# microsoft/tutel

Hardware: AMD Instinct MI355X
Metric: MoE-layer fwd tokens/sec, 4096 tok x H=2048 x E=64 top-2 (higher is better)
Workload: dtype bf16

## Files before the change

tutel_amd/csrc/expert_ffn.hip:

```cpp
#include <mutex>

#include "gemm_dev.h"

#define FFN_NQ 8
#define FFN_THREADS 256

struct FfnArgs {
  GemmArgs g[2];
  uint32_t *ctl;
  int xcc_queue;
  int prefetch;
  unsigned long long *dbg;
};

template <bool FL> static constexpr size_t ffn_lds_bytes() { return (size_t)3 * 3 * GL_STAGE * 2 + (FL ? 16384 : 16); }

template <typename V> __device__ __forceinline__ V ffn_uni(V v) {
  static_assert(sizeof(V) == 4 || sizeof(V) == 8 || sizeof(V) == 1, "scalar fields only");
  if constexpr (sizeof(V) == 8) {
    const unsigned long long b = __builtin_bit_cast(unsigned long long, v);
    const unsigned lo = (unsigned)__builtin_amdgcn_readfirstlane((int)(unsigned)b), hi = (unsigned)__builtin_amdgcn_readfirstlane((int)(b >> 32));
    return __builtin_bit_cast(V, ((unsigned long long)hi << 32) | lo);
  } else if constexpr (sizeof(V) == 4) {
    return __builtin_bit_cast(V, __builtin_amdgcn_readfirstlane(__builtin_bit_cast(int, v)));
// ... 2 lines not shown
  }
}
__device__ __forceinline__ GemmArgs ffn_pick(const GemmArgs &a0, const GemmArgs &a1, int ph) {
  GemmArgs p;
#define FFN_SEL(f) p.f = ffn_uni(ph ? a1.f : a0.f)
  FFN_SEL(A); FFN_SEL(a_stride_e); FFN_SEL(a_stride_w); FFN_SEL(a_rpw); FFN_SEL(lda);
  FFN_SEL(W); FFN_SEL(w_stride_e); FFN_SEL(ldw);
  FFN_SEL(bias); FFN_SEL(bias_stride_e);
  FFN_SEL(D); FFN_SEL(d_stride_e); FFN_SEL(d_stride_w); FFN_SEL(d_rpw); FFN_SEL(ldd);
  FFN_SEL(E_loc); FFN_SEL(R); FFN_SEL(N); FFN_SEL(K);
  FFN_SEL(row_counts); FFN_SEL(row_align);
  FFN_SEL(a_rows); FFN_SEL(a_rows_mod); FFN_SEL(a_zero); FFN_SEL(a_span_bytes);
  FFN_SEL(fits32); FFN_SEL(rot_on); FFN_SEL(sgather); FFN_SEL(d_store);
  FFN_SEL(fl_idx8); FFN_SEL(fl_n); FFN_SEL(fl_loc);
  FFN_SEL(ntm); FFN_SEL(ntn); FFN_SEL(act_rt);
#undef FFN_SEL
  p.mul = nullptr; p.d_peer = nullptr; p.d_peer_off = 0;
  p.d_can = PeerCanary{nullptr, 0, 0, 0};
  p.sk_ws = nullptr; p.sk_flags = nullptr;
  return p;
}

__device__ __forceinline__ int ffn_queue_items(int q, int E, int nt1, int nt2, int *n1) {
  const int ne = q < E ? (E - q + FFN_NQ - 1) / FFN_NQ : 0;
  *n1 = ne * nt1;
  return ne * (nt1 + nt2);
}

struct FfnTail {
  uint32_t *tick;
  int q, tid;
  int *nxt, *snap;
  int on;
  __device__ __forceinline__ void operator()() const {
// ... 166 lines not shown
  if (mode <= 0) return TUTEL_AMD_ENOTSUP;
  const int E_loc = fc1.E_loc, dtype = fc1.dtype;
  if (E_loc <= 0 || fc1.R <= 0 || fc2.dtype != dtype) return TUTEL_AMD_ENOTSUP;
  FfnArgs a;
  int rc = tutel_gemm_args(fc1, &a.g[0]);
  if (rc != 0) return rc < 0 ? rc : TUTEL_AMD_ENOTSUP;
  rc = tutel_gemm_args(fc2, &a.g[1]);
  if (rc != 0) return rc < 0 ? rc : TUTEL_AMD_ENOTSUP;
  const bool fl = fc1.fl_idx8 != nullptr;
  if (!ffn_covers(a.g[0], a.g[1])) return TUTEL_AMD_ENOTSUP;
  if (fl && !(fc1.a_rows != nullptr && fc1.fl_n >= 1 && fc1.fl_n <= 15360 && E_loc <= 128 && fc1.K >= 2 * GL_BK && ((uintptr_t)fc1.fl_idx8 & 15) == 0 &&
              tutel_get_option(TUTEL_OPT_FUSED_LOCATION) != 0))
    return TUTEL_AMD_ENOTSUP;
  if (query) return 0;
  for (int i = 0; i < 2; ++i) {
    a.g[i].ntm = 1;
    a.g[i].ntn = (a.g[i].N + 255) / 256;
  }
  a.ctl = ffn_ctl(st, E_loc);
  if (a.ctl == nullptr) return TUTEL_AMD_ENOTSUP;
  a.xcc_queue = mode == 2 ? 0 : 1;
  a.prefetch = mode == 3 ? 0 : 1;
  a.dbg = g_ffn_dbg;
  const long long items = (long long)E_loc * (a.g[0].ntn + a.g[1].ntn);
  const int cus = ffn_cus();
  const int grid = (int)(items < cus ? items : cus);
  StageScope stage(TUTEL_STAGE_FC1, st);
  TUTEL_REQUIRE(act >= TUTEL_ACT_NONE && act <= TUTEL_ACT_SILU, "tutel_amd_expert_ffn: unknown activation %d", act);
  a.g[0].act_rt = act;
  a.g[1].act_rt = TUTEL_ACT_NONE;
  if (dtype == TUTEL_BF16) return fl ? ffn_launch_cfg<bf16_t, true>(a, grid, st) : ffn_launch_cfg<bf16_t, false>(a, grid, st);
  return fl ? ffn_launch_cfg<f16_t, true>(a, grid, st) : ffn_launch_cfg<f16_t, false>(a, grid, st);
// ... 27 lines not shown
```

tutel_amd/csrc/expert_gemm.hip:

```cpp
#include <stdlib.h>

#include <mutex>
#include <type_traits>

#include "common.h"

#include "gemm_dev.h"

template <typename T, bool W_KMAJOR, int ACT, bool NT, bool ROT, bool PACKED = false>
__global__ __launch_bounds__(GM_THREADS, 2) void expert_gemm_kernel(GemmArgs p) {
  constexpr int BK = 64, NBUF = 2;
  constexpr int LDK = BK + 8;
  constexpr int A_TILE = GM_BM * LDK;
  constexpr int W_TILE = W_KMAJOR ? GM_BN * LDK : BK * GM_LDN;
  constexpr int CPR = BK / 8;
  constexpr int RPP = GM_THREADS / CPR;
  constexpr int NLA = GM_BM / RPP;
  constexpr int NLW = W_KMAJOR ? GM_BN / RPP : BK / 16;
  extern __shared__ __attribute__((aligned(16))) unsigned char smem[];
  uint16_t *sA = reinterpret_cast<uint16_t *>(smem);
  uint16_t *sW = sA + NBUF * A_TILE;

  const int tid = threadIdx.x, lane = tid & 63, wid = tid >> 6;
  const int wm = wid >> 1, wn = wid & 1;
// ... 278 lines not shown
    GL_MMA(fa[2], fw[2]);
    GL_MMA(fa[3], fw[3]);

    __syncthreads();
  }
#undef GL_ISSUE
#undef GL_LOAD_FRAGS
#undef GL_MMA

  gemm_epilogue<T, ACT>(p, acc, bias_r, e, m0, n0, wm, wn, l31, kg, row_limit);
}

template <typename T, bool W_KMAJOR, int ACT, int NI, int NS, bool BUF = false, int BM = GB_BM, bool FL = false>
__global__ __launch_bounds__(BM * 2, 2) void expert_gemm_big_kernel(GemmArgs p) {
  extern __shared__ __attribute__((aligned(16))) unsigned char smem[];
  const int w = xcd_work_item(gridDim.x);
  gemm_big_tile<T, W_KMAJOR, ACT, NI, NS, BUF, BM, FL>(p, w / (p.ntm * p.ntn), w % p.ntm, (w / p.ntm) % p.ntn, smem);
}

#define PP_BUF (4 * GL_STAGE)

template <typename T, int ACT, bool W_ONCE, bool RAGGED = false, bool EARLY_BIAS = false, bool SPLITK = false, bool PACKED = false,
          bool GATE_UP = false>
__global__ __launch_bounds__(GB_THREADS, 2) void expert_gemm_pp_kernel(GemmArgs p) {
  extern __shared__ __attribute__((aligned(16))) unsigned char smem[];
  uint16_t *lds = reinterpret_cast<uint16_t *>(smem);

  const int tid = threadIdx.x, lane = tid & 63;
  const int wid = __builtin_amdgcn_readfirstlane(tid >> 6);
  const int wm = wid >> 1, wn = wid & 1;

  static_assert(!(PACKED && SPLITK), "the packed layout never splits K");
// ... 319 lines not shown
    (void)hipGetLastError();
    if (w) (void)hipFree(w);
    if (f) (void)hipFree(f);
    return false;
  }
  e->ws = w; e->flags = f; e->tiles = tiles;
  if (e == &g_sk[g_sk_n]) ++g_sk_n;
  *ws = w;
  *flags = f;
  return true;
}

template <typename T, int ACT>
static int launch_pp_splitk(const GemmArgs &a, hipStream_t st) {
  GemmArgs b = a;
  b.ntm = (a.R + GB_BM - 1) / GB_BM;
  b.ntn = (a.N + 255) / 256;
  const size_t tiles = (size_t)b.E_loc * b.ntm * b.ntn;
  const int nk = a.K / GL_BK;
  if (a.row_counts != nullptr || a.R % GB_BM != 0 || (nk & 1) || nk < 8 || (tiles & 3) || a.rot_on) return 1;
  if ((a.ldd & 7) || (a.d_stride_e & 7) || (a.d_stride_w & 7) || (reinterpret_cast<uintptr_t>(a.D) & 15)) return 1;
  if (!splitk_workspace(st, tiles, &b.sk_ws, &b.sk_flags)) return 1;
  return launch_lds(expert_gemm_pp_kernel<T, ACT, false, false, false, true>, (unsigned)(2 * tiles), GB_THREADS, PP_LDS_BYTES, st, b,
                    "tutel_amd_expert_gemm");
}

template <typename T, int ACT>
static int launch_pp(const GemmArgs &a, hipStream_t st) {
  GemmArgs b = a;
  b.ntm = (a.R + GB_BM - 1) / GB_BM;
  b.ntn = (a.N + 255) / 256;
  const int tail_rows = b.R % GB_BM;
  const bool ragged = b.row_counts != nullptr || (tail_rows != 0 && tail_rows <= GB_BM - 32);
  const bool early = tutel_get_option(TUTEL_OPT_GEMM_PERSIST) != 0;
  if (b.ntm == 1 && (long long)b.E_loc * b.ntn >= 256)
    return ragged ? launch_pp_cfg<T, ACT, true, true>(b, st) : (early ? launch_pp_cfg<T, ACT, true, false, true>(b, st) : launch_pp_cfg<T, ACT, true>(b, st));
  return ragged ? launch_pp_cfg<T, ACT, false, true>(b, st) : (early ? launch_pp_cfg<T, ACT, false, false, true>(b, st) : launch_pp_cfg<T, ACT, false>(b, st));
}

template <typename T, int ACT>
static int launch_pp_packed(const GemmArgs &a, int tiles_bound, hipStream_t st) {
  GemmArgs b = a;
  b.ntm = 1;
  b.ntn = (a.N + 255) / 256;
  const long long grid = (long long)tiles_bound * b.ntn;
  TUTEL_REQUIRE(grid >= 1 && grid < 0x7fffffffLL, "tutel_expert_gemm_packed: grid too large");
  auto kern = (long long)a.E_loc * b.ntn >= 256 ? expert_gemm_pp_kernel<T, ACT, true, true, false, false, true>
                                                 : expert_gemm_pp_kernel<T, ACT, false, true, false, false, true>;
  return launch_lds(kern, (unsigned)grid, GB_THREADS, PP_LDS_BYTES, st, b, "tutel_expert_gemm_packed");
}

template <typename T, int ACT, bool PACKED>
static int launch_gate_up(const GemmArgs &a, int tiles_bound, hipStream_t st) {
  GemmArgs b = a;
  b.ntm = PACKED ? 1 : (a.R + GB_BM - 1) / GB_BM;
  b.ntn = (a.N + 127) / 128;
  const long long grid = PACKED ? (long long)tiles_bound * b.ntn : (long long)a.E_loc * b.ntm * b.ntn;
  TUTEL_REQUIRE(grid >= 1 && grid < 0x7fffffffLL, "tutel_amd_expert_gemm_gate_up: grid too large");
  auto kern = PACKED && (long long)a.E_loc * b.ntn >= 256 ? expert_gemm_pp_kernel<T, ACT, PACKED, true, false, false, PACKED, true>
                                                          : expert_gemm_pp_kernel<T, ACT, false, true, false, false, PACKED, true>;
  return launch_lds(kern, (unsigned)grid, GB_THREADS, PP_LDS_BYTES, st, b, "tutel_amd_expert_gemm_gate_up");
}

template <typename T, bool KM, int ACT, int NI, int NS = 2, bool BUF = false, int BM = GB_BM, bool FL = false>
static int launch_big(const GemmArgs &a, hipStream_t st) {
  GemmArgs b = a;
  b.ntm = (a.R + BM - 1) / BM;
  b.ntn = (a.N + NI * 64 - 1) / (NI * 64);
  const size_t lds_k = (size_t)NS * (BM / 128 + NI / 2) * GL_STAGE * 2 + (FL ? 16384 : 0), lds_e = BUF ? (size_t)(BM / 32) * 64 * (NI * 64 + 16) : 0;
  const size_t lds = lds_k > lds_e ? lds_k : lds_e;
  return launch_lds(expert_gemm_big_kernel<T, KM, ACT, NI, NS, BUF, BM, FL>, a.E_loc * b.ntm * b.ntn, BM * 2, lds, st, b, "tutel_amd_expert_gemm");
}

template <typename T, bool KM, int ACT>
static int launch_glds(const GemmArgs &a, int grid, hipStream_t st) {
  return launch_lds(expert_gemm_glds_kernel<T, KM, ACT, true, true>, grid, GM_THREADS, (size_t)4 * GL_STAGE * 2, st, a, "tutel_amd_expert_gemm");
}

__global__ void probe_tr16_kernel(uint16_t *out) {
  __shared__ __attribute__((aligned(16))) uint16_t lds[256];
  const int l = threadIdx.x;
  for (int i = l; i < 256; i += 64) lds[i] = (uint16_t)i;
  __syncthreads();
// ... 101 lines not shown
    const long long span = ((long long)((g.R - 1) / g.d_rows_per_w) * (g.d_stride_w < 0 ? -g.d_stride_w : g.d_stride_w) +
                            (long long)(g.d_rows_per_w < g.R ? g.d_rows_per_w : g.R) * g.ldd + g.N) * 2;
    a.d_store = (ds == 0 || span >= 0x7fffffffLL) ? 0 : (ds == 2 ? 2 : 1);
    if (g.d_peer != nullptr) {
      const long long pspan = ((long long)g.E_loc * g.d_stride_e + (long long)g.d_rows_per_w * g.ldd + g.N) * 2;
      a.d_store = (ds != 0 && g.d_rows_per_w % 8 == 0 && pspan < 0x7fffffffLL) ? 1 : 0;
    }
  }
  a.mul = g.mul;
  a.fl_idx8 = g.fl_idx8; a.fl_n = g.fl_n; a.fl_loc = g.fl_loc;
  a.d_peer = g.d_peer; a.d_peer_off = g.d_peer_off;
  a.d_can = g.d_can != nullptr ? *g.d_can : PeerCanary{nullptr, 0, 0, 0};
  TUTEL_REQUIRE(((uintptr_t)g.mul % 8) == 0, "tutel_amd_expert_gemm_glu: gating operand must be 8-byte aligned");
  TUTEL_REQUIRE(g.a_rows == nullptr || (g.a_rows_mod >= 1 && g.a_zero != nullptr && ((uintptr_t)g.a_zero % 16) == 0),
                "tutel_amd_expert_gemm_gather: need a_rows_mod >= 1 and a 16-byte aligned zero row");
  a.ntm = (g.R + GM_BM - 1) / GM_BM;
  a.ntn = (g.N + GM_BN - 1) / GM_BN;
  a.pk_off = a.pk_tiles = a.pk_ntiles = a.pk_cap = nullptr;
  a.w_up = nullptr;
  return 0;
}

int tutel_expert_gemm(const GemmProblem &g, int w_kmajor, int act, hipStream_t st) {
  TUTEL_REQUIRE(g.d_can == nullptr || g.d_peer != nullptr, "tutel_expert_gemm_peer: null peer table");
  if (g.fl_idx8 != nullptr || g.fl_loc != nullptr) {
    TUTEL_REQUIRE(g.a_rows != nullptr && g.fl_idx8 != nullptr && g.a_rows_mod >= 1 && ((uintptr_t)g.fl_idx8 & 15) == 0,
                  "tutel_expert_gemm_gather_fl: bad arguments");
    if (tutel_get_option(TUTEL_OPT_FUSED_LOCATION) == 0) return TUTEL_AMD_ENOTSUP;
  }
  GemmArgs a;
  const int brc = tutel_gemm_args(g, &a);
  if (brc != 0) return brc < 0 ? brc : 0;
  long long grid_ll = (long long)g.E_loc * a.ntm * a.ntn;
  TUTEL_REQUIRE(grid_ll < 0x7fffffffLL, "tutel_amd_expert_gemm: grid too large");
  const int grid = (int)grid_ll;
// ... 44 lines not shown
  TUTEL_REQUIRE(slot_map != nullptr && T >= 1, "tutel_amd_expert_gemm_gather: need a slot map and T >= 1");
  GemmProblem g;
  g.A = X; g.lda = ldx;
  g.W = W; g.w_stride_e = w_stride_e; g.ldw = ldw; g.bias = bias; g.bias_stride_e = bias_stride_e;
  g.D = D; g.d_stride_e = d_stride_e; g.ldd = ldd;
  g.E_loc = E_loc; g.N = N; g.K = K; g.dtype = dtype; g.row_counts = row_counts; g.row_align = row_align;
  gemm_one_rank(g, R);
  gemm_gather(g, slot_map, T, zero_row);
  return tutel_expert_gemm(g, w_kmajor, act, (hipStream_t)stream);
}


template <typename T, int ACT>
static int launch_packed_nmajor(const GemmArgs &a, int tiles_bound, hipStream_t st) {
  GemmArgs b = a;
  b.ntm = 1;
  b.ntn = (a.N + GM_BN - 1) / GM_BN;
  const long long grid = (long long)tiles_bound * 2 * b.ntn;
  TUTEL_REQUIRE(grid >= 1 && grid < 0x7fffffffLL, "tutel_amd_expert_gemm_packed: grid too large");
  return launch_lds(expert_gemm_kernel<T, false, ACT, true, true, true>, (unsigned)grid, GM_THREADS, gemm_lds_bytes(false), st, b,
                    "tutel_amd_expert_gemm_packed");
}

static int gate_up_notsup(const char *why) {
  tutel_set_error("tutel_amd_expert_gemm_gate_up: not covered: %s", why);
  return TUTEL_AMD_ENOTSUP;
}

template <bool PACKED>
static int gate_up_act(const GemmArgs &a, int dtype, int act, int tiles_bound, hipStream_t st) {
  return dispatch_dtype_act<TUTEL_ACT_RELU, TUTEL_ACT_GELU, TUTEL_ACT_SILU>(
      dtype, act, [&](auto e, auto ac) { return launch_gate_up<typename decltype(e)::type, decltype(ac)::value, PACKED>(a, tiles_bound, st); },
// ... 56 lines not shown
```

tutel_amd/csrc/gemm_dev.h:

```cpp
#pragma once
#include "common.h"

#ifndef GEMM_PROBE
#define GEMM_PROBE(i)
#endif

struct GemmArgs;
int tutel_gemm_args(const GemmProblem &g, GemmArgs *out);
bool tutel_lds_optin(const void *kern, size_t lds);

template <typename Kern, typename Args>
static int launch_lds(Kern kern, unsigned grid, int threads, size_t lds, hipStream_t st, const Args &args, const char *what) {
  if (lds > 65536 && !tutel_lds_optin((const void *)kern, lds)) return -1;
  hipLaunchKernelGGL(kern, dim3(grid), dim3(threads), lds, st, args);
  TUTEL_CHECK_LAUNCH(what);
  return 0;
}

#define GM_BM 128
#define GM_BN 128
#define GM_THREADS 256
#define GM_LDN (GM_BN + 32)

typedef __attribute__((ext_vector_type(16))) float f32x16;
// ... 28 lines not shown
}

#define GM_PRELOAD_BIAS() GM_PRELOAD_BIAS_N(2)
#define GM_PRELOAD_BIAS_N(NI_)                                                                    \
  uint2 bias_r[NI_][4];                                                                           \
  {                                                                                               \
    const uint16_t *be_ = p.bias ? reinterpret_cast<const uint16_t *>(p.bias) + (size_t)e * p.bias_stride_e : nullptr; \
    _Pragma("unroll") for (int ni_ = 0; ni_ < NI_; ++ni_)                                         \
      _Pragma("unroll") for (int rg_ = 0; rg_ < 4; ++rg_) {                                       \
        int n_ = n0 + wn * (NI_ * 32) + ni_ * 32 + rg_ * 8 + kg * 4;                              \
        n_ = n_ < p.N ? n_ : p.N - 4;                                                             \
        bias_r[ni_][rg_] = be_ ? *reinterpret_cast<const uint2 *>(be_ + n_) : make_uint2(0u, 0u); \
      }                                                                                           \
  }

struct GemmArgs {
  const void *A; long long a_stride_e, a_stride_w; int a_rpw, lda;
  const void *W; long long w_stride_e; int ldw;
  const void *bias; long long bias_stride_e;
  void *D; long long d_stride_e, d_stride_w; int d_rpw, ldd;
  int E_loc, R, N, K;
  const int32_t *row_counts; int row_align;
  const int32_t *a_rows; int a_rows_mod; const void *a_zero;
  int a_span_bytes;
  bool fits32;
  bool rot_on;
  bool sgather;
  int d_store;
  const uint8_t *fl_idx8; int fl_n; int32_t *fl_loc;
  const void *mul;
  const uint64_t *d_peer; long long d_peer_off;
  PeerCanary d_can;
  float *sk_ws; uint32_t *sk_flags;
  int ntm, ntn;
  int act_rt;
  const int32_t *pk_off, *pk_tiles, *pk_ntiles, *pk_cap;
  const void *w_up;
};

__device__ __forceinline__ uint16_t *gemm_out_row(const GemmArgs &p, int e, int m) {
  const int w = m / p.d_rpw, l = m % p.d_rpw;
  if (p.d_peer != nullptr)
    return reinterpret_cast<uint16_t *>(p.d_peer[w] + p.d_peer_off) + (size_t)e * p.d_stride_e + (size_t)l * p.ldd;
  return reinterpret_cast<uint16_t *>(p.D) + (size_t)e * p.d_stride_e + (size_t)w * p.d_stride_w + (size_t)l * p.ldd;
}

template <typename T, int ACT, int NI = 2>
__device__ __forceinline__ void gemm_epilogue(const GemmArgs &p, f32x16 (&acc)[NI][2], uint2 (&bias_r)[NI][4],
                                              int e, int m0, int n0, int wm, int wn, int l31, int kg,
                                              int row_limit) {
  uint16_t *De = reinterpret_cast<uint16_t *>(p.D) + (size_t)e * p.d_stride_e;
  const uint16_t *Me = p.mul ? reinterpret_cast<const uint16_t *>(p.mul) + (size_t)e * p.d_stride_e : nullptr;
  const bool has_bias = p.bias != nullptr;
// ... 55 lines not shown
  if (p.a_rows != nullptr) {
    const int32_t *m = p.a_rows + (size_t)e * p.R;
    const int q0 = m[gr[0]], q1 = m[gr[1]], q2 = m[gr[2]], q3 = m[gr[3]];
    q[0] = q0; q[1] = q1; q[2] = q2; q[3] = q3;
  }
}

__device__ __forceinline__ int xcd_work_item(int nb) {
  const int b = blockIdx.x, q = nb >> 3, r = nb & 7, xcd = b & 7, pos = b >> 3;
  return (xcd < r ? xcd * (q + 1) : r * (q + 1) + (xcd - r) * q) + pos;
}

__device__ __forceinline__ int padded_row_limit(const GemmArgs &p, int e) {
  int row_limit = p.R;
  if (p.row_counts != nullptr) {
    int c = p.row_counts[e];
    c = (c + p.row_align - 1) / p.row_align * p.row_align;
    row_limit = min(row_limit, c);
  }
  return row_limit;
}

template <bool NT> __device__ __forceinline__ u32x4 ld16(const uint16_t *p) {
  if (NT) return __builtin_nontemporal_load(reinterpret_cast<const u32x4 *>(p));
  return *reinterpret_cast<const u32x4 *>(p);
}

#define GL_BK 64
#define GL_STAGE (GM_BM * GL_BK)

__device__ __forceinline__ void glds16(const uint16_t *g, uint16_t *l, bool nt) {
  if (nt)
// ... 122 lines not shown
    const int row = it * RPI + r4;
    const int m = m0 + wm * 64 + row;
    const u32x4 val = *reinterpret_cast<const u32x4 *>(stage + row * PITCH + c16 * 16);
    if (m < row_limit && n < p.N) {
      const size_t roff = (size_t)(m / p.d_rpw) * p.d_stride_w + (size_t)(m % p.d_rpw) * p.ldd;
      uint16_t *drow = p.d_peer != nullptr ? gemm_out_row(p, e, m) : De + roff;
      *reinterpret_cast<u32x4 *>(drow + n) = val;
    }
  }
  if (p.d_peer != nullptr) peer_canary_store(p.d_peer, p.d_can);
}

#define GB_BM 256
#define GB_THREADS 512

struct GemmNoHook { __device__ __forceinline__ void operator()() const {} };
template <typename T, bool W_KMAJOR, int ACT, int NI, int NS, bool BUF = false, int BM = GB_BM, bool FL = false, typename Tail = GemmNoHook>
__device__ __forceinline__ void gemm_big_tile(const GemmArgs &p, const int e, const int mt, const int nt, unsigned char *smem,
                                              Tail tail = Tail()) {
  static_assert(!FL || (BUF && NS == 3 && BM == 128 && W_KMAJOR), "FL: the 128 x 256 ring kernel only");
  constexpr int NW = BM / 32;
  constexpr int NSUB = NI / 2;
  constexpr int WPW = 16 * NSUB / NW;
  constexpr int BN = NI * 64;
  constexpr int A_STAGE = (BM / 128) * GL_STAGE;
  uint16_t *sA = reinterpret_cast<uint16_t *>(smem);
  uint16_t *sW = sA + NS * A_STAGE;

  const int tid = threadIdx.x, lane = tid & 63;
  const int wid = __builtin_amdgcn_readfirstlane(tid >> 6);
  const int wm = wid >> 1, wn = wid & 1;
  const int wsub = (wn * NI * 32) / GM_BN, wcol = (wn * NI * 32) % GM_BN;

  const int m0 = mt * BM, n0 = nt * BN;
  GEMM_PROBE(0);

  const int row_limit = padded_row_limit(p, e);
  if (m0 >= row_limit) {
    tail();
    return;
  }

  const uint16_t *Ae = reinterpret_cast<const uint16_t *>(p.A) + (size_t)e * p.a_stride_e;
  const uint16_t *We = reinterpret_cast<const uint16_t *>(p.W) + (size_t)e * p.w_stride_e;

  const uint16_t *a_src[4], *w_src[WPW];
  int gr4[4], slot4[4];
  constexpr bool SG = BUF && NS == 3;
  typedef int sgv8u __attribute__((ext_vector_type(8), aligned(4)));
  sgv8u sg_q[4];
  const bool fl_on = FL && p.fl_idx8 != nullptr;
  const int mo_ = e * p.R + m0 + 32 * wid;
  const bool sg_on = SG && p.a_rows != nullptr && p.sgather && !fl_on && mo_ + 32 <= p.E_loc * p.R;
#pragma unroll
  for (int i = 0; i < 4; ++i) gr4[i] = min(m0 + 8 * (wid * 4 + i) + (lane >> 3), p.R - 1);
  if (!sg_on && !fl_on) gather_rows4(p, e, gr4, slot4);
#define GB_A_ADDR()                                                                                             \
  _Pragma("unroll") for (int i = 0; i < 4; ++i) {                                                              \
    const int r = 8 * (wid * 4 + i) + (lane >> 3);                                                             \
    const int c = (lane & 7) ^ ((r >> 1) & 7);                                                                 \
    const int gr = gr4[i];                                                                                     \
    a_src[i] = Ae + (size_t)(gr / p.a_rpw) * p.a_stride_w + (size_t)(gr % p.a_rpw) * p.lda + c * 8;            \
    if (p.a_rows != nullptr) {                                                                                 \
      const int q = slot4[i];                                                                                  \
      a_src[i] = (q >= 0 ? reinterpret_cast<const uint16_t *>(p.A) + (size_t)(q % p.a_rows_mod) * p.lda        \
                         : reinterpret_cast<const uint16_t *>(p.a_zero)) + c * 8;                              \
    }                                                                                                          \
  }
  if (!sg_on && !fl_on) { GB_A_ADDR(); }
#pragma unroll
  for (int i = 0; i < WPW; ++i) {
    const int g = wid * WPW + i, dg = g >> 4, j = g & 15;
    if (W_KMAJOR) {
      const int r = 8 * j + (lane >> 3);
      const int c = (lane & 7) ^ ((r >> 1) & 7);
      const int gn = min(n0 + dg * GM_BN + r, p.N - 1);
      w_src[i] = We + (size_t)gn * p.ldw + c * 8;
    } else {
      const int kr = 4 * j + (lane >> 4);
      const int cn = (lane & 15) ^ ((kr & 3) << 2);
      const int gn = min(n0 + dg * GM_BN + cn * 8, p.N - 8);
      w_src[i] = We + (size_t)kr * p.ldw + gn;
    }
  }
  const size_t w_step = W_KMAJOR ? (size_t)GL_BK : (size_t)GL_BK * p.ldw;
  const int piece_a = wid * 4 * 512, piece_w = wid * WPW * 512;
  int a_off[4], w_off[WPW];
  const uint16_t *abase = p.a_rows != nullptr ? reinterpret_cast<const uint16_t *>(p.A) : Ae;
#define GB_A_OFF()                                                                                              \
  _Pragma("unroll") for (int i = 0; i < 4; ++i) {                                                              \
    const int r = 8 * (wid * 4 + i) + (lane >> 3);                                                             \
    a_off[i] = (int)(unsigned)((const char *)a_src[i] - (const char *)abase);                                  \
    if ((p.a_rows != nullptr && slot4[i] < 0) || m0 + r >= row_limit)                                          \
      a_off[i] = (int)0x7ffff000u + (((lane & 7) ^ ((r >> 1) & 7)) << 4);   \
  }
  if (BUF) {
    if (!sg_on && !fl_on) { GB_A_OFF(); }
#pragma unroll
    for (int i = 0; i < WPW; ++i) w_off[i] = (int)(unsigned)((const char *)w_src[i] - (const char *)We);
  }
  const __amdgpu_buffer_rsrc_t rs_a = __builtin_amdgcn_make_buffer_rsrc(
      const_cast<uint16_t *>(p.a_rows != nullptr ? reinterpret_cast<const uint16_t *>(p.A) : Ae), 0, p.a_span_bytes, 0x00020000);
  const __amdgpu_buffer_rsrc_t rs_w = __builtin_amdgcn_make_buffer_rsrc(const_cast<uint16_t *>(We), 0, -1, 0x00020000);
  const bool w_once = NI == 4 && p.ntm == 1 && gridDim.x >= 256;

  f32x16 acc[NI][2];
#pragma unroll
  for (int i = 0; i < NI; ++i)
#pragma unroll
    for (int j = 0; j < 2; ++j)
#pragma unroll
      for (int r = 0; r < 16; ++r) acc[i][j][r] = 0.f;

  const int l31 = lane & 31, kg = lane >> 5;
  const int sw = (l31 >> 1) & 7;
  int frag_k[4];
#pragma unroll
  for (int kk = 0; kk < 4; ++kk) frag_k[kk] = (((kk * 2 + kg) ^ sw) << 3);
  const int a_row = (wm * 64 + l31) * GL_BK;
  const int wk_row = (wcol + l31) * GL_BK;
  const int g16 = lane >> 4, i16 = lane & 15, q4 = i16 >> 2;
  const int c_lo = wcol / 8 + (g16 & 1) * 2 + ((i16 & 3) >> 1);
  const int wt_row = ((g16 >> 1) * 8 + q4) * GM_BN;
  int wt_c[NI];
#pragma unroll
  for (int ni = 0; ni < NI; ++ni) wt_c[ni] = (((c_lo + 4 * ni) ^ (q4 << 2)) << 3) + (i16 & 1) * 4;

  const int nk = p.K / GL_BK;
  const int npair = NI == 4 ? p.ntn : (p.ntn + 1) >> 1, pair = NI == 4 ? nt : nt >> 1;
  const int rot = p.rot_on ? (int)(((long long)(pair + 3 * e) * nk / npair) % nk) : 0;

#define GB_ISSUE_A(KT, STG)                                                            \
  do {                                                                                 \
    int kr_ = (KT) + rot; kr_ = kr_ >= nk ? kr_ - nk : kr_;                            \
    uint16_t *da_ = sA + (STG) * A_STAGE + piece_a;                                    \
    if (BUF) {                                                                         \
      const int ao_ = kr_ * (GL_BK * 2);                                               \
      _Pragma("unroll") for (int i_ = 0; i_ < 4; ++i_) bdma16<false>(rs_a, a_off[i_], ao_, da_ + i_ * 512); \
    } else {                                                                           \
      const size_t ao_ = (size_t)kr_ * GL_BK;                                          \
      _Pragma("unroll") for (int i_ = 0; i_ < 4; ++i_) glds16(a_src[i_] + ao_, da_ + i_ * 512, false); \
    }                                                                                  \
  } while (0)
#define GB_ISSUE_W(KT, STG)                                                            \
  do {                                                                                 \
// ... 53 lines not shown
    GB_MMA(fa[1], fw[1]);                                                              \
  } while (0)

  if (NS == 2) {
    GB_ISSUE(0, 0);
    __syncthreads();
    for (int kt = 0; kt < nk; ++kt) {
      const int buf = kt & 1;
      if (kt + 1 < nk) GB_ISSUE(kt + 1, buf ^ 1);
      GB_TILE(buf);
      __syncthreads();
    }
  } else {
    constexpr int OPS = 4 + WPW;
    static_assert(NS <= 3, "the prologue order below is worked out for rings of at most three slots");
    constexpr int FL_CH = 4;
    unsigned char *s_fl = smem + (size_t)NS * (A_STAGE + NSUB * GL_STAGE) * 2;
    if (FL && fl_on) {
      static_assert(!FL || WPW * (NS - 1) == 16, "the vmcnt(16) of the fused-location prologue counts the weight ops of the first two tiles");
      const __amdgpu_buffer_rsrc_t rs_i = __builtin_amdgcn_make_buffer_rsrc(const_cast<uint8_t *>(p.fl_idx8), 0, (p.fl_n + 15) & ~15, 0x00020000);
      const int per_ = (((p.fl_n + 255) >> 8) + 15) & ~15, ipw = per_ >> 4;
      for (int i = wid * ipw; i < (wid + 1) * ipw; ++i)
        if (i < 15) bdma16<false>(rs_i, i * 1024 + lane * 16, 0, reinterpret_cast<uint16_t *>(s_fl + i * 1024));
    }
    if (sg_on) {
      asm volatile("" ::"s"(reinterpret_cast<uintptr_t>(We)), "s"(rot), "s"(nk), "s"((int)w_once), "s"((int)(w_step * 2)));
#pragma unroll
      for (int i = 0; i < WPW; ++i) asm volatile("" ::"v"(w_off[i]));
      const __attribute__((address_space(4))) sgv8u *mp =
          reinterpret_cast<const __attribute__((address_space(4))) sgv8u *>(reinterpret_cast<uintptr_t>(p.a_rows) + (size_t)mo_ * 4);
#pragma unroll
      for (int i = 0; i < 4; ++i) sg_q[i] = mp[i];
    }
#pragma unroll
    for (int t = 0; t < NS - 1; ++t)
      if (t < nk) GB_ISSUE_W(t, t);
    if (sg_on) {
      const int rl_ = lane >> 3;
#pragma unroll
      for (int i = 0; i < 4; ++i) {
        int q = sg_q[i][0];
#pragma unroll
        for (int j = 1; j < 8; ++j) q = (rl_ == j) ? sg_q[i][j] : q;
        slot4[i] = q;
      }
      GB_A_ADDR();
      GB_A_OFF();
    }
    if (FL && fl_on) {
      int *s_slot = reinterpret_cast<int *>(s_fl + 15360);
      int *s_wt = s_slot + 128;
// ... 57 lines not shown
              if (first_tile) p.fl_loc[q] = r;
              if (r < p.R) s_slot[r] = q;
              ++r;
              t &= t - 1;
            }
          }
      }
      asm volatile("s_waitcnt lgkmcnt(0)" ::: "memory");
      __builtin_amdgcn_s_barrier();
      asm volatile("" ::: "memory");
#pragma unroll
      for (int i = 0; i < 4; ++i) slot4[i] = s_slot[8 * (wid * 4 + i) + (lane >> 3)];
      if (first_tile && tid < p.R) const_cast<int32_t *>(p.a_rows)[(size_t)e * p.R + tid] = s_slot[tid];
      GB_A_ADDR();
      GB_A_OFF();
    }
#pragma unroll
    for (int t = 0; t < NS - 1; ++t)
      if (t < nk) GB_ISSUE_A(t, t);
    int kt = 0, slot = 0;
    GEMM_PROBE(1);
    for (; kt + NS - 1 < nk; ++kt) {
      if (kt == 0) asm volatile("s_waitcnt vmcnt(%0)" ::"n"(4 * (NS - 2)) : "memory");
      else asm volatile("s_waitcnt vmcnt(%0)" ::"n"(OPS * (NS - 2)) : "memory");
      __builtin_amdgcn_s_barrier();
      if (kt == 0) { GEMM_PROBE(2); }
      const int nslot = slot == 0 ? NS - 1 : slot - 1;
      GB_ISSUE(kt + NS - 1, nslot);
      GB_TILE(slot);
      slot = slot + 1 == NS ? 0 : slot + 1;
    }
    GEMM_PROBE(3);
    for (; kt < nk; ++kt) {
      asm volatile("s_waitcnt vmcnt(0)" ::: "memory");
      __builtin_amdgcn_s_barrier();
      GB_TILE(slot);
      slot = slot + 1 == NS ? 0 : slot + 1;
    }
    GEMM_PROBE(4);
  }
#undef GB_TILE
#undef GB_A_ADDR
#undef GB_A_OFF
#undef GB_ISSUE
#undef GB_ISSUE_A
#undef GB_ISSUE_W
#undef GB_LOAD_FRAGS
#undef GB_MMA

  tail();
  GM_PRELOAD_BIAS_N(NI);
  if (BUF && !((p.ldd & 7) || (p.d_stride_e & 7) || (p.d_stride_w & 7) || (reinterpret_cast<uintptr_t>(p.D) & 15))) {
    __syncthreads();
    unsigned char *stage = smem + wid * (64 * (NI * 64 + 16));
    if (ACT == GEMM_ACT_RUNTIME) {
      if (p.act_rt == TUTEL_ACT_NONE) gemm_epilogue_lds<T, TUTEL_ACT_NONE, NI>(p, acc, bias_r, stage, e, m0, n0, wm, wn, lane, row_limit);
      else if (p.act_rt == TUTEL_ACT_RELU) gemm_epilogue_lds<T, TUTEL_ACT_RELU, NI>(p, acc, bias_r, stage, e, m0, n0, wm, wn, lane, row_limit);
// ... 12 lines not shown
```

Baseline: 16.87 million.

## Reorder GemmArgs head, precompute magic divisors, defer kernarg loads past weight DMA

Reorders GemmArgs so the fields needed to start the weight DMA sit in the first kernarg cache lines. Integer divisions and modulos by tile counts, row_align, a_rpw and a_rows_mod are replaced with host-precomputed multiply-high magic constants. In the 3-stage ring path, the A-side argument loads and address setup are deferred until after the first weight DMAs are issued, to shorten the kernel prologue. This adds complexity and inline-asm register pinning, and changes the rot formula, which risks subtle numeric or indexing differences.

```diff
diff --git a/tutel_amd/csrc/expert_ffn.hip b/tutel_amd/csrc/expert_ffn.hip
--- a/tutel_amd/csrc/expert_ffn.hip
+++ b/tutel_amd/csrc/expert_ffn.hip
@@ -40,10 +40,13 @@
   FFN_SEL(fits32); FFN_SEL(rot_on); FFN_SEL(sgather); FFN_SEL(d_store);
   FFN_SEL(fl_idx8); FFN_SEL(fl_n); FFN_SEL(fl_loc);
   FFN_SEL(ntm); FFN_SEL(ntn); FFN_SEL(act_rt);
+  FFN_SEL(ntm_d.mul); FFN_SEL(ntm_d.sh); FFN_SEL(ntn_d.mul); FFN_SEL(ntn_d.sh); FFN_SEL(npair_d.mul); FFN_SEL(npair_d.sh);
+  FFN_SEL(row_align_d.mul); FFN_SEL(row_align_d.sh); FFN_SEL(a_rpw_d.mul); FFN_SEL(a_rpw_d.sh); FFN_SEL(a_rows_mod_d.mul); FFN_SEL(a_rows_mod_d.sh);
 #undef FFN_SEL
   p.mul = nullptr; p.d_peer = nullptr; p.d_peer_off = 0;
   p.d_can = PeerCanary{nullptr, 0, 0, 0};
   p.sk_ws = nullptr; p.sk_flags = nullptr;
+  p.pk_off = p.pk_tiles = p.pk_ntiles = p.pk_cap = nullptr; p.w_up = nullptr;
   return p;
 }
 
@@ -240,8 +243,7 @@
     return TUTEL_AMD_ENOTSUP;
   if (query) return 0;
   for (int i = 0; i < 2; ++i) {
-    a.g[i].ntm = 1;
-    a.g[i].ntn = (a.g[i].N + 255) / 256;
+    gemm_set_tiles(a.g[i], 1, (a.g[i].N + 255) / 256);
   }
   a.ctl = ffn_ctl(st, E_loc);
   if (a.ctl == nullptr) return TUTEL_AMD_ENOTSUP;
diff --git a/tutel_amd/csrc/expert_gemm.hip b/tutel_amd/csrc/expert_gemm.hip
--- a/tutel_amd/csrc/expert_gemm.hip
+++ b/tutel_amd/csrc/expert_gemm.hip
@@ -316,8 +316,9 @@
 template <typename T, bool W_KMAJOR, int ACT, int NI, int NS, bool BUF = false, int BM = GB_BM, bool FL = false>
 __global__ __launch_bounds__(BM * 2, 2) void expert_gemm_big_kernel(GemmArgs p) {
   extern __shared__ __attribute__((aligned(16))) unsigned char smem[];
-  const int w = xcd_work_item(gridDim.x);
-  gemm_big_tile<T, W_KMAJOR, ACT, NI, NS, BUF, BM, FL>(p, w / (p.ntm * p.ntn), w % p.ntm, (w / p.ntm) % p.ntn, smem);
+  const int w = xcd_work_item((int)gemm_head_fetch(p));
+  const int t = (int)divu((uint32_t)w, p.ntm_d), e = (int)divu((uint32_t)t, p.ntn_d);
+  gemm_big_tile<T, W_KMAJOR, ACT, NI, NS, BUF, BM, FL, GemmNoHook, true>(p, e, w - t * p.ntm, t - e * p.ntn, smem);
 }
 
 #define PP_BUF (4 * GL_STAGE)
@@ -667,8 +668,7 @@
 template <typename T, int ACT>
 static int launch_pp_splitk(const GemmArgs &a, hipStream_t st) {
   GemmArgs b = a;
-  b.ntm = (a.R + GB_BM - 1) / GB_BM;
-  b.ntn = (a.N + 255) / 256;
+  gemm_set_tiles(b, (a.R + GB_BM - 1) / GB_BM, (a.N + 255) / 256);
   const size_t tiles = (size_t)b.E_loc * b.ntm * b.ntn;
   const int nk = a.K / GL_BK;
   if (a.row_counts != nullptr || a.R % GB_BM != 0 || (nk & 1) || nk < 8 || (tiles & 3) || a.rot_on) return 1;
@@ -681,8 +681,7 @@
 template <typename T, int ACT>
 static int launch_pp(const GemmArgs &a, hipStream_t st) {
   GemmArgs b = a;
-  b.ntm = (a.R + GB_BM - 1) / GB_BM;
-  b.ntn = (a.N + 255) / 256;
+  gemm_set_tiles(b, (a.R + GB_BM - 1) / GB_BM, (a.N + 255) / 256);
   const int tail_rows = b.R % GB_BM;
   const bool ragged = b.row_counts != nullptr || (tail_rows != 0 && tail_rows <= GB_BM - 32);
   const bool early = tutel_get_option(TUTEL_OPT_GEMM_PERSIST) != 0;
@@ -694,8 +693,7 @@
 template <typename T, int ACT>
 static int launch_pp_packed(const GemmArgs &a, int tiles_bound, hipStream_t st) {
   GemmArgs b = a;
-  b.ntm = 1;
-  b.ntn = (a.N + 255) / 256;
+  gemm_set_tiles(b, 1, (a.N + 255) / 256);
   const long long grid = (long long)tiles_bound * b.ntn;
   TUTEL_REQUIRE(grid >= 1 && grid < 0x7fffffffLL, "tutel_expert_gemm_packed: grid too large");
   auto kern = (long long)a.E_loc * b.ntn >= 256 ? expert_gemm_pp_kernel<T, ACT, true, true, false, false, true>
@@ -706,8 +704,7 @@
 template <typename T, int ACT, bool PACKED>
 static int launch_gate_up(const GemmArgs &a, int tiles_bound, hipStream_t st) {
   GemmArgs b = a;
-  b.ntm = PACKED ? 1 : (a.R + GB_BM - 1) / GB_BM;
-  b.ntn = (a.N + 127) / 128;
+  gemm_set_tiles(b, PACKED ? 1 : (a.R + GB_BM - 1) / GB_BM, (a.N + 127) / 128);
   const long long grid = PACKED ? (long long)tiles_bound * b.ntn : (long long)a.E_loc * b.ntm * b.ntn;
   TUTEL_REQUIRE(grid >= 1 && grid < 0x7fffffffLL, "tutel_amd_expert_gemm_gate_up: grid too large");
   auto kern = PACKED && (long long)a.E_loc * b.ntn >= 256 ? expert_gemm_pp_kernel<T, ACT, PACKED, true, false, false, PACKED, true>
@@ -718,8 +715,7 @@
 template <typename T, bool KM, int ACT, int NI, int NS = 2, bool BUF = false, int BM = GB_BM, bool FL = false>
 static int launch_big(const GemmArgs &a, hipStream_t st) {
   GemmArgs b = a;
-  b.ntm = (a.R + BM - 1) / BM;
-  b.ntn = (a.N + NI * 64 - 1) / (NI * 64);
+  gemm_set_tiles(b, (a.R + BM - 1) / BM, (a.N + NI * 64 - 1) / (NI * 64));
   const size_t lds_k = (size_t)NS * (BM / 128 + NI / 2) * GL_STAGE * 2 + (FL ? 16384 : 0), lds_e = BUF ? (size_t)(BM / 32) * 64 * (NI * 64 + 16) : 0;
   const size_t lds = lds_k > lds_e ? lds_k : lds_e;
   return launch_lds(expert_gemm_big_kernel<T, KM, ACT, NI, NS, BUF, BM, FL>, a.E_loc * b.ntm * b.ntn, BM * 2, lds, st, b, "tutel_amd_expert_gemm");
@@ -851,11 +847,22 @@
   TUTEL_REQUIRE(((uintptr_t)g.mul % 8) == 0, "tutel_amd_expert_gemm_glu: gating operand must be 8-byte aligned");
   TUTEL_REQUIRE(g.a_rows == nullptr || (g.a_rows_mod >= 1 && g.a_zero != nullptr && ((uintptr_t)g.a_zero % 16) == 0),
                 "tutel_amd_expert_gemm_gather: need a_rows_mod >= 1 and a 16-byte aligned zero row");
-  a.ntm = (g.R + GM_BM - 1) / GM_BM;
-  a.ntn = (g.N + GM_BN - 1) / GM_BN;
+  gemm_set_tiles(a, (g.R + GM_BM - 1) / GM_BM, (g.N + GM_BN - 1) / GM_BN);
+  TUTEL_REQUIRE((long long)((g.N + 255) / 256) * (g.K / 64) < 0x7fffffffLL, "tutel_amd_expert_gemm: N=%d x K=%d too large", g.N, g.K);
+  TUTEL_REQUIRE(g.row_counts == nullptr || (long long)g.R + a.row_align < 0x7fffffffLL, "tutel_amd_expert_gemm: R + row_align too large");
+  a.npair_d = divu_make((uint32_t)((g.N + 255) / 256));
+  a.row_align_d = divu_make((uint32_t)a.row_align);
+  a.a_rpw_d = divu_make((uint32_t)a.a_rpw);
+  a.a_rows_mod_d = divu_make((uint32_t)(a.a_rows_mod < 0 ? 0 : a.a_rows_mod));
+  a.sk_ws = nullptr; a.sk_flags = nullptr; a.act_rt = TUTEL_ACT_NONE;
   a.pk_off = a.pk_tiles = a.pk_ntiles = a.pk_cap = nullptr;
   a.w_up = nullptr;
   return 0;
+}
+
+extern "C" void tutel_divu_probe(uint32_t d, uint32_t *mul, uint32_t *sh) {
+  const DivU c = divu_make(d);
+  *mul = c.mul; *sh = c.sh;
 }
 
 int tutel_expert_gemm(const GemmProblem &g, int w_kmajor, int act, hipStream_t st) {
@@ -930,8 +937,7 @@
 template <typename T, int ACT>
 static int launch_packed_nmajor(const GemmArgs &a, int tiles_bound, hipStream_t st) {
   GemmArgs b = a;
-  b.ntm = 1;
-  b.ntn = (a.N + GM_BN - 1) / GM_BN;
+  gemm_set_tiles(b, 1, (a.N + GM_BN - 1) / GM_BN);
   const long long grid = (long long)tiles_bound * 2 * b.ntn;
   TUTEL_REQUIRE(grid >= 1 && grid < 0x7fffffffLL, "tutel_amd_expert_gemm_packed: grid too large");
   return launch_lds(expert_gemm_kernel<T, false, ACT, true, true, true>, (unsigned)grid, GM_THREADS, gemm_lds_bytes(false), st, b,
diff --git a/tutel_amd/csrc/gemm_dev.h b/tutel_amd/csrc/gemm_dev.h
--- a/tutel_amd/csrc/gemm_dev.h
+++ b/tutel_amd/csrc/gemm_dev.h
@@ -1,4 +1,5 @@
 #pragma once
+#include <cstddef>
 #include "common.h"
 
 #ifndef GEMM_PROBE
@@ -66,29 +67,51 @@
       }                                                                                           \
   }
 
+struct DivU { uint32_t mul, sh; };
+inline DivU divu_make(uint32_t d) {
+  DivU c = {0u, 0u};
+  if (d < 2) return c;
+  uint32_t l = 0;
+  while ((1ull << l) < d) ++l;
+  c.mul = (uint32_t)((((unsigned long long)1 << (31 + l)) + d - 1) / d);
+  c.sh = l - 1;
+  return c;
+}
+__device__ __forceinline__ uint32_t divu(uint32_t n, const DivU &c) { return c.mul ? __umulhi(n, c.mul) >> c.sh : n; }
+
 struct GemmArgs {
+  const void *W; long long w_stride_e; int ldw, N, K, R;
+  int E_loc, ntm, ntn;
+  int rot_on;
+  DivU ntm_d, ntn_d;
+  DivU npair_d;
+  int sgather;
+  int row_align; const int32_t *row_counts; DivU row_align_d;
+  const int32_t *a_rows;
+  const uint8_t *fl_idx8; int fl_n;
+  int fits32;
+  DivU a_rpw_d;
+  DivU a_rows_mod_d;
   const void *A; long long a_stride_e, a_stride_w; int a_rpw, lda;
-  const void *W; long long w_stride_e; int ldw;
+  int a_rows_mod; int a_span_bytes;
+  const void *a_zero;
   const void *bias; long long bias_stride_e;
   void *D; long long d_stride_e, d_stride_w; int d_rpw, ldd;
-  int E_loc, R, N, K;
-  const int32_t *row_counts; int row_align;
-  const int32_t *a_rows; int a_rows_mod; const void *a_zero;
-  int a_span_bytes;
-  bool fits32;
-  bool rot_on;
-  bool sgather;
   int d_store;
-  const uint8_t *fl_idx8; int fl_n; int32_t *fl_loc;
+  int32_t *fl_loc;
   const void *mul;
   const uint64_t *d_peer; long long d_peer_off;
   PeerCanary d_can;
   float *sk_ws; uint32_t *sk_flags;
-  int ntm, ntn;
   int act_rt;
   const int32_t *pk_off, *pk_tiles, *pk_ntiles, *pk_cap;
   const void *w_up;
 };
+static_assert(offsetof(GemmArgs, a_rows_mod_d) == 128 && offsetof(GemmArgs, bias) <= 192, "GemmArgs: the head is two 64-byte lines, the token-row addressing a third");
+inline void gemm_set_tiles(GemmArgs &a, int ntm, int ntn) {
+  a.ntm = ntm; a.ntn = ntn;
+  a.ntm_d = divu_make((uint32_t)ntm); a.ntn_d = divu_make((uint32_t)ntn);
+}
 
 __device__ __forceinline__ uint16_t *gemm_out_row(const GemmArgs &p, int e, int m) {
   const int w = m / p.d_rpw, l = m % p.d_rpw;
@@ -174,8 +197,9 @@
 __device__ __forceinline__ int padded_row_limit(const GemmArgs &p, int e) {
   int row_limit = p.R;
   if (p.row_counts != nullptr) {
-    int c = p.row_counts[e];
-    c = (c + p.row_align - 1) / p.row_align * p.row_align;
+    const int cnt = *reinterpret_cast<const __attribute__((address_space(4))) int32_t *>(reinterpret_cast<uintptr_t>(p.row_counts + e));
+    const int c0 = min(max(cnt, 0), p.R);
+    const int c = (int)(divu((uint32_t)(c0 + p.row_align - 1), p.row_align_d) * (uint32_t)p.row_align);
     row_limit = min(row_limit, c);
   }
   return row_limit;
@@ -328,9 +352,41 @@
 #define GB_BM 256
 #define GB_THREADS 512
 
+#define GEMM_HEAD_REGS(p)                                                                                                          \
+  "s"(reinterpret_cast<uintptr_t>((p).W)), "s"((p).w_stride_e), "s"((p).ldw), "s"((p).N), "s"((p).K), "s"((p).R), "s"((p).E_loc),    \
+      "s"((p).ntm), "s"((p).ntn), "s"((p).rot_on), "s"((p).ntm_d.mul), "s"((p).ntm_d.sh), "s"((p).ntn_d.mul), "s"((p).ntn_d.sh),     \
+      "s"((p).npair_d.mul), "s"((p).npair_d.sh), "s"((p).sgather), "s"((p).row_align), "s"(reinterpret_cast<uintptr_t>((p).row_counts)), \
+      "s"((p).row_align_d.mul), "s"((p).row_align_d.sh), "s"(reinterpret_cast<uintptr_t>((p).a_rows)),                              \
+      "s"(reinterpret_cast<uintptr_t>((p).fl_idx8)), "s"((p).fl_n)
+__device__ __forceinline__ unsigned gemm_head_fetch(const GemmArgs &p) {
+  unsigned nb = gridDim.x;
+  asm volatile("" : "+s"(nb) : GEMM_HEAD_REGS(p));
+  return nb;
+}
 struct GemmNoHook { __device__ __forceinline__ void operator()() const {} };
-template <typename T, bool W_KMAJOR, int ACT, int NI, int NS, bool BUF = false, int BM = GB_BM, bool FL = false, typename Tail = GemmNoHook>
-__device__ __forceinline__ void gemm_big_tile(const GemmArgs &p, const int e, const int mt, const int nt, unsigned char *smem,
+template <bool KARG> __device__ __forceinline__ void gemm_args_late(GemmArgs &q, const GemmArgs &ph) {
+  q = ph;
+  if (KARG) {
+    uintptr_t ka = reinterpret_cast<uintptr_t>(__builtin_amdgcn_kernarg_segment_ptr());
+    asm volatile("" : "+s"(ka));
+    const __attribute__((address_space(4))) GemmArgs *k = reinterpret_cast<const __attribute__((address_space(4))) GemmArgs *>(ka);
+#define GB_LATE(f) q.f = k->f
+    GB_LATE(a_rows_mod_d.mul); GB_LATE(a_rows_mod_d.sh);
+    GB_LATE(A); GB_LATE(a_stride_e); GB_LATE(a_stride_w); GB_LATE(a_rpw); GB_LATE(lda);
+    GB_LATE(bias); GB_LATE(bias_stride_e);
+    GB_LATE(D); GB_LATE(d_stride_e); GB_LATE(d_stride_w); GB_LATE(d_rpw); GB_LATE(ldd);
+    GB_LATE(a_rows_mod); GB_LATE(a_zero); GB_LATE(a_span_bytes); GB_LATE(d_store); GB_LATE(fl_loc); GB_LATE(mul);
+    GB_LATE(d_peer); GB_LATE(d_peer_off); GB_LATE(d_can.epoch); GB_LATE(d_can.off); GB_LATE(d_can.world); GB_LATE(d_can.stale);
+    GB_LATE(sk_ws); GB_LATE(sk_flags); GB_LATE(act_rt);
+    GB_LATE(pk_off); GB_LATE(pk_tiles); GB_LATE(pk_ntiles); GB_LATE(pk_cap); GB_LATE(w_up);
+#undef GB_LATE
+    asm volatile("" ::"s"(q.a_rows_mod_d.mul), "s"(q.a_rows_mod_d.sh), "s"(reinterpret_cast<uintptr_t>(q.A)), "s"(q.a_stride_e), "s"(q.a_stride_w),
+                 "s"(q.a_rpw), "s"(q.lda), "s"(q.a_rows_mod), "s"(q.a_span_bytes), "s"(reinterpret_cast<uintptr_t>(q.a_zero)));
+  }
+}
+template <typename T, bool W_KMAJOR, int ACT, int NI, int NS, bool BUF = false, int BM = GB_BM, bool FL = false, typename Tail = GemmNoHook,
+          bool KARG = false>
+__device__ __forceinline__ void gemm_big_tile(const GemmArgs &ph, const int e, const int mt, const int nt, unsigned char *smem,
                                               Tail tail = Tail()) {
   static_assert(!FL || (BUF && NS == 3 && BM == 128 && W_KMAJOR), "FL: the 128 x 256 ring kernel only");
   constexpr int NW = BM / 32;
@@ -349,58 +405,82 @@
   const int m0 = mt * BM, n0 = nt * BN;
   GEMM_PROBE(0);
 
-  const int row_limit = padded_row_limit(p, e);
+  constexpr bool A_LATE = NS == 3;
+  if (A_LATE) asm volatile("" ::GEMM_HEAD_REGS(ph));
+  GEMM_PROBE(6);
+
+  const int row_limit = padded_row_limit(ph, e);
   if (m0 >= row_limit) {
     tail();
     return;
   }
 
-  const uint16_t *Ae = reinterpret_cast<const uint16_t *>(p.A) + (size_t)e * p.a_stride_e;
-  const uint16_t *We = reinterpret_cast<const uint16_t *>(p.W) + (size_t)e * p.w_stride_e;
+  constexpr bool SG = BUF && NS == 3;
+  const bool fl_on = FL && ph.fl_idx8 != nullptr;
+  constexpr int FL_CH = 4;
+  unsigned char *s_fl = smem + (size_t)NS * (A_STAGE + NSUB * GL_STAGE) * 2;
+  if (FL && fl_on) {
+    static_assert(!FL || WPW * (NS - 1) == 16, "the vmcnt(16) of the fused-location prologue counts the weight ops of the first two tiles");
+    const __amdgpu_buffer_rsrc_t rs_i = __builtin_amdgcn_make_buffer_rsrc(const_cast<uint8_t *>(ph.fl_idx8), 0, (ph.fl_n + 15) & ~15, 0x00020000);
+    const int per_ = (((ph.fl_n + 255) >> 8) + 15) & ~15, ipw = per_ >> 4;
+    for (int i = wid * ipw; i < (wid + 1) * ipw; ++i)
+      if (i < 15) bdma16<false>(rs_i, i * 1024 + lane * 16, 0, reinterpret_cast<uint16_t *>(s_fl + i * 1024));
+  }
+  GemmArgs pl_;
+  const GemmArgs &p = A_LATE ? pl_ : ph;
+  const uint16_t *We = reinterpret_cast<const uint16_t *>(ph.W) + (size_t)e * ph.w_stride_e;
+  const uint16_t *Ae, *abase;
+  __amdgpu_buffer_rsrc_t rs_a;
+#define GB_A_BASE()                                                                                             \
+  do {                                                                                                          \
+    Ae = reinterpret_cast<const uint16_t *>(p.A) + (size_t)e * p.a_stride_e;                                    \
+    abase = p.a_rows != nullptr ? reinterpret_cast<const uint16_t *>(p.A) : Ae;                                 \
+    rs_a = __builtin_amdgcn_make_buffer_rsrc(const_cast<uint16_t *>(abase), 0, p.a_span_bytes, 0x00020000);     \
+  } while (0)
+  if (!A_LATE) { GB_A_BASE(); }
 
   const uint16_t *a_src[4], *w_src[WPW];
   int gr4[4], slot4[4];
-  constexpr bool SG = BUF && NS == 3;
   typedef int sgv8u __attribute__((ext_vector_type(8), aligned(4)));
   sgv8u sg_q[4];
-  const bool fl_on = FL && p.fl_idx8 != nullptr;
-  const int mo_ = e * p.R + m0 + 32 * wid;
-  const bool sg_on = SG && p.a_rows != nullptr && p.sgather && !fl_on && mo_ + 32 <= p.E_loc * p.R;
-#pragma unroll
-  for (int i = 0; i < 4; ++i) gr4[i] = min(m0 + 8 * (wid * 4 + i) + (lane >> 3), p.R - 1);
-  if (!sg_on && !fl_on) gather_rows4(p, e, gr4, slot4);
+  const int mo_ = e * ph.R + m0 + 32 * wid;
+  const bool sg_on = SG && ph.a_rows != nullptr && ph.sgather && !fl_on && mo_ + 32 <= ph.E_loc * ph.R;
+#pragma unroll
+  for (int i = 0; i < 4; ++i) gr4[i] = min(m0 + 8 * (wid * 4 + i) + (lane >> 3), ph.R - 1);
+  if (!sg_on && !fl_on) gather_rows4(ph, e, gr4, slot4);
 #define GB_A_ADDR()                                                                                             \
   _Pragma("unroll") for (int i = 0; i < 4; ++i) {                                                              \
     const int r = 8 * (wid * 4 + i) + (lane >> 3);                                                             \
     const int c = (lane & 7) ^ ((r >> 1) & 7);                                                                 \
     const int gr = gr4[i];                                                                                     \
-    a_src[i] = Ae + (size_t)(gr / p.a_rpw) * p.a_stride_w + (size_t)(gr % p.a_rpw) * p.lda + c * 8;            \
+    const int gw = (int)divu((uint32_t)gr, p.a_rpw_d);                                                         \
+    a_src[i] = Ae + (size_t)gw * p.a_stride_w + (size_t)(gr - gw * p.a_rpw) * p.lda + c * 8;                   \
     if (p.a_rows != nullptr) {                                                                                 \
       const int q = slot4[i];                                                                                  \
-      a_src[i] = (q >= 0 ? reinterpret_cast<const uint16_t *>(p.A) + (size_t)(q % p.a_rows_mod) * p.lda        \
+      const int qt = q - (int)divu((uint32_t)q, p.a_rows_mod_d) * p.a_rows_mod;     \
+      a_src[i] = (q >= 0 ? reinterpret_cast<const uint16_t *>(p.A) + (size_t)qt * p.lda                        \
                          : reinterpret_cast<const uint16_t *>(p.a_zero)) + c * 8;                              \
     }                                                                                                          \
   }
-  if (!sg_on && !fl_on) { GB_A_ADDR(); }
+  if (!A_LATE && !sg_on && !fl_on) { GB_A_ADDR(); }
 #pragma unroll
   for (int i = 0; i < WPW; ++i) {
     const int g = wid * WPW + i, dg = g >> 4, j = g & 15;
     if (W_KMAJOR) {
       const int r = 8 * j + (lane >> 3);
       const int c = (lane & 7) ^ ((r >> 1) & 7);
-      const int gn = min(n0 + dg * GM_BN + r, p.N - 1);
-      w_src[i] = We + (size_t)gn * p.ldw + c * 8;
+      const int gn = min(n0 + dg * GM_BN + r, ph.N - 1);
+      w_src[i] = We + (size_t)gn * ph.ldw + c * 8;
     } else {
       const int kr = 4 * j + (lane >> 4);
       const int cn = (lane & 15) ^ ((kr & 3) << 2);
-      const int gn = min(n0 + dg * GM_BN + cn * 8, p.N - 8);
-      w_src[i] = We + (size_t)kr * p.ldw + gn;
-    }
-  }
-  const size_t w_step = W_KMAJOR ? (size_t)GL_BK : (size_t)GL_BK * p.ldw;
+      const int gn = min(n0 + dg * GM_BN + cn * 8, ph.N - 8);
+      w_src[i] = We + (size_t)kr * ph.ldw + gn;
+    }
+  }
+  const size_t w_step = W_KMAJOR ? (size_t)GL_BK : (size_t)GL_BK * ph.ldw;
   const int piece_a = wid * 4 * 512, piece_w = wid * WPW * 512;
   int a_off[4], w_off[WPW];
-  const uint16_t *abase = p.a_rows != nullptr ? reinterpret_cast<const uint16_t *>(p.A) : Ae;
 #define GB_A_OFF()                                                                                              \
   _Pragma("unroll") for (int i = 0; i < 4; ++i) {                                                              \
     const int r = 8 * (wid * 4 + i) + (lane >> 3);                                                             \
@@ -409,14 +489,12 @@
       a_off[i] = (int)0x7ffff000u + (((lane & 7) ^ ((r >> 1) & 7)) << 4);   \
   }
   if (BUF) {
-    if (!sg_on && !fl_on) { GB_A_OFF(); }
+    if (!A_LATE && !sg_on && !fl_on) { GB_A_OFF(); }
 #pragma unroll
     for (int i = 0; i < WPW; ++i) w_off[i] = (int)(unsigned)((const char *)w_src[i] - (const char *)We);
   }
-  const __amdgpu_buffer_rsrc_t rs_a = __builtin_amdgcn_make_buffer_rsrc(
-      const_cast<uint16_t *>(p.a_rows != nullptr ? reinterpret_cast<const uint16_t *>(p.A) : Ae), 0, p.a_span_bytes, 0x00020000);
   const __amdgpu_buffer_rsrc_t rs_w = __builtin_amdgcn_make_buffer_rsrc(const_cast<uint16_t *>(We), 0, -1, 0x00020000);
-  const bool w_once = NI == 4 && p.ntm == 1 && gridDim.x >= 256;
+  const bool w_once = NI == 4 && ph.ntm == 1 && gridDim.x >= 256;
 
   f32x16 acc[NI][2];
 #pragma unroll
@@ -440,9 +518,13 @@
 #pragma unroll
   for (int ni = 0; ni < NI; ++ni) wt_c[ni] = (((c_lo + 4 * ni) ^ (q4 << 2)) << 3) + (i16 & 1) * 4;
 
-  const int nk = p.K / GL_BK;
-  const int npair = NI == 4 ? p.ntn : (p.ntn + 1) >> 1, pair = NI == 4 ? nt : nt >> 1;
-  const int rot = p.rot_on ? (int)(((long long)(pair + 3 * e) * nk / npair) % nk) : 0;
+  const int nk = ph.K / GL_BK;
+  const int npair = NI == 4 ? ph.ntn : (ph.ntn + 1) >> 1, pair = NI == 4 ? nt : nt >> 1;
+  int rot = 0;
+  if (ph.rot_on) {
+    const uint32_t x = (uint32_t)(pair + 3 * e), b = x - divu(x, ph.npair_d) * (uint32_t)npair;
+    rot = (int)divu(b * (uint32_t)nk, ph.npair_d);
+  }
 
 #define GB_ISSUE_A(KT, STG)                                                            \
   do {                                                                                 \
@@ -526,27 +608,26 @@
   } else {
     constexpr int OPS = 4 + WPW;
     static_assert(NS <= 3, "the prologue order below is worked out for rings of at most three slots");
-    constexpr int FL_CH = 4;
-    unsigned char *s_fl = smem + (size_t)NS * (A_STAGE + NSUB * GL_STAGE) * 2;
-    if (FL && fl_on) {
-      static_assert(!FL || WPW * (NS - 1) == 16, "the vmcnt(16) of the fused-location prologue counts the weight ops of the first two tiles");
-      const __amdgpu_buffer_rsrc_t rs_i = __builtin_amdgcn_make_buffer_rsrc(const_cast<uint8_t *>(p.fl_idx8), 0, (p.fl_n + 15) & ~15, 0x00020000);
-      const int per_ = (((p.fl_n + 255) >> 8) + 15) & ~15, ipw = per_ >> 4;
-      for (int i = wid * ipw; i < (wid + 1) * ipw; ++i)
-        if (i < 15) bdma16<false>(rs_i, i * 1024 + lane * 16, 0, reinterpret_cast<uint16_t *>(s_fl + i * 1024));
-    }
     if (sg_on) {
       asm volatile("" ::"s"(reinterpret_cast<uintptr_t>(We)), "s"(rot), "s"(nk), "s"((int)w_once), "s"((int)(w_step * 2)));
 #pragma unroll
       for (int i = 0; i < WPW; ++i) asm volatile("" ::"v"(w_off[i]));
       const __attribute__((address_space(4))) sgv8u *mp =
-          reinterpret_cast<const __attribute__((address_space(4))) sgv8u *>(reinterpret_cast<uintptr_t>(p.a_rows) + (size_t)mo_ * 4);
+          reinterpret_cast<const __attribute__((address_space(4))) sgv8u *>(reinterpret_cast<uintptr_t>(ph.a_rows) + (size_t)mo_ * 4);
 #pragma unroll
       for (int i = 0; i < 4; ++i) sg_q[i] = mp[i];
     }
+    asm volatile("; gemm_big_tile: first weight DMA");
 #pragma unroll
     for (int t = 0; t < NS - 1; ++t)
       if (t < nk) GB_ISSUE_W(t, t);
+    GEMM_PROBE(7);
+    gemm_args_late<KARG>(pl_, ph);
+    GB_A_BASE();
+    if (A_LATE && !sg_on && !fl_on) {
+      GB_A_ADDR();
+      if (BUF) { GB_A_OFF(); }
+    }
     if (sg_on) {
       const int rl_ = lane >> 3;
 #pragma unroll
@@ -634,6 +715,7 @@
       if (first_tile && tid < p.R) const_cast<int32_t *>(p.a_rows)[(size_t)e * p.R + tid] = s_slot[tid];
       GB_A_ADDR();
       GB_A_OFF();
+      GEMM_PROBE(8);
     }
 #pragma unroll
     for (int t = 0; t < NS - 1; ++t)
@@ -661,6 +743,7 @@
   }
 #undef GB_TILE
 #undef GB_A_ADDR
+#undef GB_A_BASE
 #undef GB_A_OFF
 #undef GB_ISSUE
 #undef GB_ISSUE_A
```

Result: no change. 16.96 million, median of 5 (+0.5%).
